# Nicolo2277/Vivim

Hardware: AMD Instinct MI355X
Metric: frames/sec fwd+bwd, 256x256 clip=5 3-class (higher is better)
Workload: dtype bf16

## Files before the change

### vivim_amd/csrc/scan_bwd.hip

```cpp
#include "scan_plan.cuh"

namespace vivim {

constexpr int kBwdWaves = 4;

template <typename T, int K, int R, bool HAS_Z, bool VAR_BC, bool DET = false>
__global__ void __launch_bounds__(kBwdWaves * kWave) ssm_bwd_generic_kernel(const vivim_ssm_bwd_params p, const int ck) {
    constexpr int TILE = kWave * K;
    const vivim_ssm_fwd_params& f = p.f;
    const int lane = threadIdx.x & 63;
    const int wave = threadIdx.x >> 6;
    const int b = blockIdx.y;
    const int N = f.dstate, L = f.seqlen;
    const int cpg = f.dim / f.n_groups;
    const int wpg = (cpg + R - 1) / R;
    const int ws = blockIdx.x * kBwdWaves + wave;
    if (ws >= wpg * f.n_groups) return;
    const int g = ws / wpg;
    const int d0 = g * cpg + (ws - g * wpg) * R;
    const int nvalid = min(R, (g + 1) * cpg - d0);

    extern __shared__ __attribute__((aligned(16))) float smem[];
    constexpr bool FOLD_BC = DET && !VAR_BC;
    float* gcarry = smem + wave * (FOLD_BC ? 5 : 3) * R * N;
// ... 394 lines not shown
                    H = f2{H0, H1};
                }
                {
                    const f2 hend = fma2(P, hck, H);
                    f2 h = dpp_mov2<kDppWaveShr1>(hck, hend);
#pragma unroll
                    for (int k = 0; k < K; ++k) {
                        h = fma2(a[k], h, wB[k]);
                        hs[k] = h;
                    }
                }
                const f2 an = dpp_mov2<kDppWaveShl1>(afirst, a[0]);
                f2 cdy[K], Pr = an, G = {0.0f, 0.0f};
#pragma unroll
                for (int k = K - 1; k >= 0; --k) {
                    const f2 al = k == K - 1 ? an : a[k + 1];
                    cdy[k] = dy[k] * Cn[k];
                    G = fma2(al, G, cdy[k]);
                    if (k < K - 1) Pr *= al;
                }
                f2 gfirst;
                {
                    float P0 = Pr.x, G0 = G.x, P1 = Pr.y, G1 = G.y;
                    wave_scan2_affine_rev_rows(P0, G0, P1, G1);
                    wave_scan_rev_join(P0, G0, lane);
                    wave_scan_rev_join(P1, G1, lane);
                    gfirst = fma2(f2{P0, P1}, gcar, f2{G0, G1});
                }
                f2 gc = dpp_mov2<kDppWaveShl1>(gcar, gfirst);
                f2 dA_part = {0.0f, 0.0f};
                float dBv[K], dCv[K];
#pragma unroll
                for (int k = K - 1; k >= 0; --k) {
                    const f2 al = k == K - 1 ? an : a[k + 1];
                    gc = fma2(al, gc, cdy[k]);
                    const f2 t = gc * (hs[k] - wB[k]);
                    S1[k] = fma2(gc, f2{Bn[k], Bn[k]}, S1[k]);
                    S2[k] = fma2(t, a2v, S2[k]);
                    dA_part = fma2(t, dl[k], dA_part);
                    const f2 db = gc * w[k], dc = dy[k] * hs[k];
                    dBv[k] = db.x + db.y;
                    dCv[k] = dc.x + dc.y;
                }
                if (DA_LDS) {
                    dAl[n * kWave + lane] += dA_part;
                    if (lane == 0) {
                        f2* qq = reinterpret_cast<f2*>(rec + n * kRec * R);
                        qq[GCAR] = gfirst;
                        qq[AFIRST] = a[0];
                    }
                } else {
                    const float dA0 = read_lane(wave_sum_dpp_to63(dA_part.x), 63);
                    const float dA1 = read_lane(wave_sum_dpp_to63(dA_part.y), 63);
                    if (lane == 0) {
                        f2* qq = reinterpret_cast<f2*>(rec + n * kRec * R);
                        qq[GCAR] = gfirst;
                        qq[AFIRST] = a[0];
                        qq[DAACC] += f2{dA0, dA1};
                    }
                }
                {
                    float* sl = slots + ((n & (NBUF - 1)) * W + wave) * SLOT + lane;
#pragma unroll
                    for (int k = 0; k < K; ++k) {
                        sl[k * kWave] = dBv[k];
                        sl[(K + k) * kWave] = dCv[k];
                    }
                }
                lds_barrier();
#pragma unroll
                for (int j = 0; j < EPT; ++j) {
                    const int e = tid + j * (W * kWave);
                    const int e_tok = e & (TILE - 1), e_isC = e / TILE;
                    const float* sp = slots + (n & (NBUF - 1)) * W * SLOT +
                                      (e_isC * K + (e_tok & (K - 1))) * kWave + (e_tok / K);
                    float acc = sp[0];
#pragma unroll
                    for (int wv = 1; wv < W; ++wv) acc += sp[wv * SLOT];
                    const int tq = step * TILE + e_tok;
                    const int t = tq < L ? tq : tq % L;
                    if (DET) {
                        if (tq < L) (e_isC ? dCg + n * p.dC_dstate_stride : dBg + n * p.dB_dstate_stride)[tq] = acc;
                        continue;
                    }
                    atomicAdd((e_isC ? dCg + n * p.dC_dstate_stride : dBg + n * p.dB_dstate_stride) + t, acc);
                }
            }
        }
#pragma unroll
        for (int r = 0; r < R; ++r) {
            float duv[K], ddv[K], uu[K];
            unpack(load_vec_always<T, K>(uB + d[r] * f.u_d_stride + t0, in, uB + d[r] * f.u_d_stride), uu);
#pragma unroll
            for (int k = 0; k < K; ++k) {
                duv[k] = fmaf(dl[k][r], S1[k][r], Dv[r] * dy[k][r]);
                ddv[k] = fmaf(uu[k], S1[k][r], S2[k][r] * kLn2);
            }
            if (f.delta_softplus) {
                float df[K];
                unpack(load_vec_always<T, K>(dlB + d[r] * f.delta_d_stride + t0, in, dlB + d[r] * f.delta_d_stride), df);
#pragma unroll
                for (int k = 0; k < K; ++k) {
                    const float raw = df[k] + bias[r];
                    if (raw <= 20.0f) ddv[k] *= sigmoidf_fast(raw);
                }
            }
#pragma unroll
            for (int k = 0; k < K; ++k) dbias_acc[r] += in ? ddv[k] : 0.0f;
            store_vec<T, K>(static_cast<T*>(p.du) + b * p.du_batch_stride + d[r] * p.du_d_stride + t0, in && active && r < nvalid, duv);
            store_vec<T, K>(static_cast<T*>(p.ddelta) + b * p.ddelta_batch_stride + d[r] * p.ddelta_d_stride + t0, in && active && r < nvalid, ddv);
        }
    }
    if (active) {
#pragma unroll
        for (int r = 0; r < R; ++r) {
            if (r >= nvalid) break;
            const float sD = wave_sum(dD_acc[r]);
            const float sb = wave_sum(dbias_acc[r]);
            if (lane == 0) {
                const int64_t slot = DET ? (int64_t)(b * gridDim.z + seg) * f.dim : 0;
                if (p.dD) det_add<DET>(static_cast<float*>(p.dD) + slot + d[r], sD);
                if (p.ddelta_bias) det_add<DET>(static_cast<float*>(p.ddelta_bias) + slot + d[r], sb);
            }
        }
        wave_lds_fence();
        for (int i = lane; i < N * R; i += kWave) {
            const int n = i / R, r = i - n * R;
            float tot = VIVIM_REC(n, DAACC, r);
            if (DA_LDS) {
                const float* q = reinterpret_cast<const float*>(dAl + n * kWave) + r;
                tot = 0.0f;
                for (int j = 0; j < kWave; ++j) tot += q[j * R];
            }
            if (r < nvalid)
                det_add<DET>(static_cast<float*>(p.dA) + (DET ? (int64_t)(b * gridDim.z + seg) * f.dim * N : 0) +
                             (d0 + r) * p.dA_d_stride + n * p.dA_dstate_stride, tot);
        }
    }
#undef VIVIM_REC
}

constexpr int kPreW = 4;
template <typename T, int K, bool HAS_Z, int NS>
__global__ void __launch_bounds__(kPreW * kWave) ssm_bwd_prepass_kernel(const vivim_ssm_bwd_params p, const BwdSeg sg) {
    constexpr int R = kBwR;
    constexpr int TILE = kWave * K;
    const vivim_ssm_fwd_params& f = p.f;
    const int lane = threadIdx.x & 63;
    const int wave = __builtin_amdgcn_readfirstlane(threadIdx.x >> 6);
    const int b = blockIdx.y;
    const int N = f.dstate, L = f.seqlen;
    const int cpg = f.dim / f.n_groups;
    const int ppg = (cpg + R - 1) / R;
    const int nw = blockDim.x >> 6;
    const int bpg = (ppg + nw - 1) / nw;
    const int g = blockIdx.x / bpg;
    const int pair = (blockIdx.x - g * bpg) * nw + wave;
    if (pair >= ppg) return;
    const int d0 = g * cpg + pair * R;
    const int nvalid = min(R, (g + 1) * cpg - d0);
    const int nsteps = (L + TILE - 1) / TILE;
    const int seg = blockIdx.z + 1;
    const int s_lo = seg * sg.seg_steps, s_hi = min(nsteps, s_lo + sg.seg_steps);
    const int t_next = s_hi * TILE;

    extern __shared__ __attribute__((aligned(16))) float smem[];
    float* acc = smem + wave * (N * R * kWave);
    if (NS == 0)
        for (int i = lane; i < N * R * kWave; i += kWave) acc[i] = 0.0f;
    f2 racc[NS > 0 ? NS : 1];
#pragma unroll
    for (int n = 0; n < (NS > 0 ? NS : 1); ++n) racc[n] = f2{0.0f, 0.0f};

    int d[R];
    float bias[R], a2v[R];
#pragma unroll
    for (int r = 0; r < R; ++r) {
        d[r] = d0 + min(r, nvalid - 1);
        bias[r] = f.delta_bias ? static_cast<const float*>(f.delta_bias)[d[r]] : 0.0f;
        a2v[r] = lane < N ? static_cast<const float*>(f.A)[d[r] * f.A_d_stride + lane * f.A_dstate_stride] * kLog2e : 0.0f;
    }
    const T* __restrict__ dlB = static_cast<const T*>(f.delta) + b * f.delta_batch_stride;
    const T* __restrict__ doB = static_cast<const T*>(p.dout) + b * p.dout_batch_stride;
    const T* __restrict__ zB = HAS_Z ? static_cast<const T*>(f.z) + b * f.z_batch_stride : nullptr;
    const T* __restrict__ Cv = static_cast<const T*>(f.C) + b * f.C_batch_stride + g * f.C_group_stride;
    wave_lds_fence();

    float base[R] = {0.0f, 0.0f}, dfirst[R] = {0.0f, 0.0f};
    RawK<T, K> ndl[R], ndo[R], nz[R];
    auto request = [&](int step) __attribute__((always_inline)) {
        const int t0 = step * TILE + lane * K;
        const bool in = step < s_hi && t0 < L;
#pragma unroll
        for (int r = 0; r < R; ++r) {
            ndl[r] = load_vec_always<T, K>(dlB + d[r] * f.delta_d_stride + t0, in, dlB + d[r] * f.delta_d_stride);
            ndo[r] = load_vec_always<T, K>(doB + d[r] * p.dout_d_stride + t0, in, doB + d[r] * p.dout_d_stride);
            if (HAS_Z) nz[r] = load_vec_always<T, K>(zB + d[r] * f.z_d_stride + t0, in, zB + d[r] * f.z_d_stride);
        }
    };
    constexpr bool kAhead = sizeof(T) * K <= 16;
    if (kAhead) request(s_lo);
    for (int step = s_lo; step < s_hi; ++step) {
        const int t0 = step * TILE + lane * K;
        const bool in = t0 < L;
        float c[R][K], dy[R][K];
        RawK<T, K> cdl[R], cdo[R], cz[R];
        if (!kAhead) request(step);
#pragma unroll
        for (int r = 0; r < R; ++r) { cdl[r] = ndl[r]; cdo[r] = ndo[r]; if (HAS_Z) cz[r] = nz[r]; }
        if (kAhead) request(step + 1);
#pragma unroll
        for (int r = 0; r < R; ++r) {
            float df[K];
            unpack(cdl[r], df);
            unpack(cdo[r], dy[r]);
            if (HAS_Z) {
                float zf[K];
                unpack(cz[r], zf);
#pragma unroll
                for (int k = 0; k < K; ++k) dy[r][k] *= zf[k] * sigmoidf_fast(zf[k]);
            }
            float run = 0.0f;
#pragma unroll
            for (int k = 0; k < K; ++k) {
                const float raw = df[k] + bias[r];
                const float sp = f.delta_softplus ? softplus_ref(raw) : raw;
                run += in ? sp : 0.0f;
                c[r][k] = run;
            }
            if (step == s_lo) {
                dfirst[r] = read_lane(c[r][0], 0);
                base[r] = -dfirst[r];
            }
            const float incl = wave_sum_dpp_to63(run);
            const float off = incl - run + base[r];
#pragma unroll
            for (int k = 0; k < K; ++k) c[r][k] += off;
            base[r] += read_lane(incl, 63);
        }
        RawK<T, K> Craw = load_vec_always<T, K>(Cv + t0, in, Cv);
        if (NS > 0) {
            f2 cp[K], dyp[K];
#pragma unroll
            for (int k = 0; k < K; ++k) { cp[k] = f2{c[0][k], c[1][k]}; dyp[k] = f2{dy[0][k], dy[1][k]}; }
#pragma unroll
            for (int n = 0; n < NS; ++n) {
                float Cn[K];
                unpack(Craw, Cn);
                Craw = load_vec_always<T, K>(Cv + (n + 1) * f.C_dstate_stride + t0, in && (n + 1 < NS), Cv);
                const f2 A2 = {read_lane(a2v[0], n), read_lane(a2v[1], n)};
#pragma unroll
                for (int k = 0; k < K; ++k) racc[n] = fma2(exp2_2(A2 * cp[k]), dyp[k] * Cn[k], racc[n]);
            }
        } else {
#pragma unroll 1
            for (int n = 0; n < N; ++n) {
                float Cn[K];
                unpack(Craw, Cn);
                Craw = load_vec_always<T, K>(Cv + (n + 1) * f.C_dstate_stride + t0, in && (n + 1 < N), Cv);
#pragma unroll
                for (int r = 0; r < R; ++r) {
                    const float A2 = read_lane(a2v[r], n);
                    float* q = acc + (n * R + r) * kWave + lane;
                    float v = *q;
#pragma unroll
                    for (int k = 0; k < K; ++k) v = fmaf(fast_exp2(A2 * c[r][k]), Cn[k] * dy[r][k], v);
                    *q = v;
                }
            }
        }
    }
    if (NS > 0) {
#pragma unroll
        for (int n = 0; n < NS; ++n) {
            acc[(n * R + 0) * kWave + lane] = racc[n].x;
            acc[(n * R + 1) * kWave + lane] = racc[n].y;
        }
    }
    wave_lds_fence();
    for (int row0 = 0; row0 < N * R; row0 += kWave / 2) {
        const int row = row0 + (lane >> 1);
        float v = 0.0f;
        if (row < N * R) {
            const float* q = acc + row * kWave + (lane & 1) * (kWave / 2);
#pragma unroll 8
            for (int j = 0; j < kWave / 2; ++j) v += q[j];
        }
        v += __shfl_xor(v, 1, kWave);
        const int n = row / R, r = row - n * R;
        if (row < N * R && (lane & 1) == 0 && r < nvalid)
            sg.agg[(((int64_t)b * f.dim + d0 + r) * sg.S + seg) * N + n] = v;
    }
#pragma unroll
    for (int r = 0; r < R; ++r) {
        float dl_nx = 0.0f;
        if (t_next < L) {
            const float raw = to_f32<T>((dlB + d[r] * f.delta_d_stride)[t_next]) + bias[r];
            dl_nx = f.delta_softplus ? softplus_ref(raw) : raw;
        }
        if (lane == 0 && r < nvalid) sg.dsum[((int64_t)b * f.dim + d[r]) * sg.S + seg] = base[r] + dl_nx;
    }
}

__global__ void ssm_bwd_carry_kernel(const vivim_ssm_bwd_params p, const BwdSeg sg) {
    const vivim_ssm_fwd_params& f = p.f;
    const int64_t i = (int64_t)blockIdx.x * blockDim.x + threadIdx.x;
    const int N = f.dstate;
    if (i >= (int64_t)f.batch * f.dim * N) return;
    const int n = (int)(i % N);
    const int64_t bd = i / N;
    const int dch = (int)(bd % f.dim);
    const float A2 = static_cast<const float*>(f.A)[dch * f.A_d_stride + n * f.A_dstate_stride] * kLog2e;
    float g = 0.0f;
    const int S = sg.S;
    sg.gin[(bd * S + S - 1) * N + n] = 0.0f;
    for (int i0 = 0; i0 < S - 1; i0 += 8) {
        float ag[8], ds[8];
#pragma unroll
        for (int q = 0; q < 8; ++q) {
            const int s = S - 1 - (i0 + q);
            const bool ok = s >= 1;
            ag[q] = ok ? sg.agg[(bd * S + s) * N + n] : 0.0f;
            ds[q] = ok ? sg.dsum[bd * S + s] : 0.0f;
        }
#pragma unroll
        for (int q = 0; q < 8; ++q) {
            const int s = S - 1 - (i0 + q);
            if (s >= 1) {
                g = fmaf(fast_exp2(A2 * ds[q]), g, ag[q]);
                sg.gin[(bd * S + s - 1) * N + n] = g;
            }
        }
    }
}

template <typename T, int K, int DS>
static void launch_prepass(const vivim_ssm_bwd_params& p, const BwdSeg& sg, hipStream_t stream) {
    const vivim_ssm_fwd_params& f = p.f;
    const int ppg = (f.dim / f.n_groups + kBwR - 1) / kBwR;
    const size_t per_wave = (size_t)f.dstate * kBwR * kWave * sizeof(float);
    int nw = (int)((size_t)65536 / per_wave);
    nw = nw > kPreW ? kPreW : (nw < 1 ? 1 : nw);
    const dim3 gpre(((ppg + nw - 1) / nw) * f.n_groups, f.batch, sg.S - 1);
    if (f.z) hipLaunchKernelGGL((ssm_bwd_prepass_kernel<T, K, true, DS>), gpre, dim3(nw * kWave), nw * per_wave, stream, p, sg);
    else     hipLaunchKernelGGL((ssm_bwd_prepass_kernel<T, K, false, DS>), gpre, dim3(nw * kWave), nw * per_wave, stream, p, sg);
    const int64_t nthr = (int64_t)f.batch * f.dim * f.dstate;
    hipLaunchKernelGGL(ssm_bwd_carry_kernel, dim3((unsigned)((nthr + 255) / 256)), dim3(256), 0, stream, p, sg);
}

void launch_bwd_closed_prepass(const vivim_ssm_bwd_params& p, const LsSeg& ls, int K, hipStream_t stream) {
    const BwdSeg sg = {ls.S, ls.seg_blocks * 16 / (K * kWave), ls.agg, ls.dsum, ls.gin};
    with_itype(p.f.itype, [&](auto t) {
        typedef decltype(t) T;
        if (K == 8) launch_prepass<T, 8, 16>(p, sg, stream); else launch_prepass<T, 4, 16>(p, sg, stream);
    });
}

template <typename T, int K, int W, bool DET>
static void launch_bwd_fast_kw(const vivim_ssm_bwd_params& p, const BwdPlan& q, hipStream_t stream) {
    const vivim_ssm_fwd_params& f = p.f;
    const int ppg = (f.dim / f.n_groups + kBwR - 1) / kBwR;
    const int bpg = (ppg + W - 1) / W;
    BwdSeg sg = {q.S, q.seg, nullptr, nullptr, nullptr};
    if (q.S > 1) {
        const size_t nbd = (size_t)f.batch * f.dim * sg.S;
        sg.agg = static_cast<float*>(p.workspace);
        sg.gin = sg.agg + nbd * f.dstate;
        sg.dsum = sg.gin + nbd * f.dstate;
        if (f.dstate == 16) launch_prepass<T, K, 16>(p, sg, stream);
        else                launch_prepass<T, K, 0>(p, sg, stream);
    }
    const size_t smem = ((size_t)2 * W * 2 * K * kWave + (size_t)W * f.dstate * kBwR * kRec +
                         (q.da_lds ? (size_t)W * f.dstate * kWave * 2 : 0)) * sizeof(float);
    const dim3 grid(bpg * f.n_groups, f.batch, sg.S), block(W * kWave);
    auto launch = [&](auto kernel) {
        allow_smem(kernel, smem);
        hipLaunchKernelGGL(kernel, grid, block, smem, stream, p, sg);
    };
    if (f.z) { if (q.da_lds) launch(ssm_bwd_fast_kernel<T, K, true, W, true, DET>); else launch(ssm_bwd_fast_kernel<T, K, true, W, false, DET>); }
    else     { if (q.da_lds) launch(ssm_bwd_fast_kernel<T, K, false, W, true, DET>); else launch(ssm_bwd_fast_kernel<T, K, false, W, false, DET>); }
}

template <bool DET>
static void launch_bwd_fast_t(const vivim_ssm_bwd_params& p, const BwdPlan& q, hipStream_t stream) {
    with_itype(p.f.itype, [&](auto t) {
        typedef decltype(t) T;
        if (q.K == 8) {
            if constexpr (DET) launch_bwd_fast_kw<T, 8, 4, DET>(p, q, stream);
            else if (q.W == 4) launch_bwd_fast_kw<T, 8, 4, DET>(p, q, stream);
            else               launch_bwd_fast_kw<T, 8, kBwWmax, DET>(p, q, stream);
        }
        else          { if (q.W == 4) launch_bwd_fast_kw<T, 4, 4, DET>(p, q, stream); else launch_bwd_fast_kw<T, 4, kBwWmax, DET>(p, q, stream); }
    });
}
void launch_bwd_fast(const vivim_ssm_bwd_params& p, const BwdPlan& q, hipStream_t stream, bool det) {
    if (det) launch_bwd_fast_t<true>(p, q, stream); else launch_bwd_fast_t<false>(p, q, stream);
}

template <bool DET>
static void launch_bwd_generic_t(const vivim_ssm_bwd_params& p, int ck, hipStream_t stream) {
    constexpr int K = 4, R = kBwdGenR;
    const vivim_ssm_fwd_params& f = p.f;
    const int sets = ((f.dim / f.n_groups + R - 1) / R) * f.n_groups;
    const dim3 grid((sets + kBwdWaves - 1) / kBwdWaves, f.batch), block(kBwdWaves * kWave);
    const bool var = f.is_variable_B;
    const size_t smem = (size_t)kBwdWaves * (DET && !var ? 5 : 3) * R * f.dstate * sizeof(float);
    with_itype(f.itype, [&](auto t) {
        typedef decltype(t) T;
        if (f.z) {
            if (var) hipLaunchKernelGGL((ssm_bwd_generic_kernel<T, K, R, true, true, DET>), grid, block, smem, stream, p, ck);
            else     hipLaunchKernelGGL((ssm_bwd_generic_kernel<T, K, R, true, false, DET>), grid, block, smem, stream, p, ck);
        } else {
            if (var) hipLaunchKernelGGL((ssm_bwd_generic_kernel<T, K, R, false, true, DET>), grid, block, smem, stream, p, ck);
            else     hipLaunchKernelGGL((ssm_bwd_generic_kernel<T, K, R, false, false, DET>), grid, block, smem, stream, p, ck);
        }
    });
}
void launch_bwd_generic(const vivim_ssm_bwd_params& p, int ck, hipStream_t stream, bool det) {
    if (det) launch_bwd_generic_t<true>(p, ck, stream); else launch_bwd_generic_t<false>(p, ck, stream);
}

}
```

### vivim_amd/csrc/scan_plan.hip

```cpp
#include <stdlib.h>
#include <algorithm>
#include <atomic>
#include "scan_plan.cuh"

namespace vivim {

const ScanEnv& scan_env() {
    static const ScanEnv e = [] {
        auto num = [](const char* name, int dflt) { const char* v = getenv(name); return v ? atoi(v) : dflt; };
        return ScanEnv{num("VIVIM_CHAN_WAVES", 2048), num("VIVIM_CHAN_XCD", -1)};
    }();
    return e;
}

static int cu_count() {
    static const int n = [] {
        int dev = 0, v = 0;
        if (hipGetDevice(&dev) != hipSuccess ||
            hipDeviceGetAttribute(&v, hipDeviceAttributeMultiprocessorCount, dev) != hipSuccess || v <= 0)
            v = 256;
        return v;
    }();
    return n;
}

static int ls_bwd_blocks_per_cu(const vivim_ssm_fwd_params& f, int W, bool ls2) {
    static std::atomic<int> cache[2][3][3][2][5];
    if (f.itype < 0 || f.itype > 2) return ls2 ? 2 : 3;
    std::atomic<int>& c = cache[ls2][f.itype][f.dstate / 32][f.z != nullptr][W];
    int nb = c.load(std::memory_order_relaxed);
    if (nb == 0) {
        nb = ls2 ? ls2_bwd_occupancy(f, W) : ls_bwd_occupancy(f, W);
        c.store(nb, std::memory_order_relaxed);
    }
    return nb;
}

static bool rows_vec_ok(const void* ptr, std::initializer_list<int64_t> strides, int64_t epv, int es) {
    if (reinterpret_cast<uintptr_t>(ptr) % (uintptr_t)(epv * es)) return false;
    for (int64_t s : strides)
        if (s % epv) return false;
    return true;
}
static int esize(int itype) { return itype == VIVIM_F32 ? 4 : 2; }
static int epv16(int itype) { return 16 / esize(itype); }
static bool fwd_rows_vec_ok(const vivim_ssm_fwd_params& f, int64_t epv, bool ptrs = true) {
    const int es = esize(f.itype);
    auto P = [&](const void* q) { return ptrs ? q : nullptr; };
    return rows_vec_ok(P(f.u), {f.u_batch_stride, f.u_d_stride}, epv, es) &&
           rows_vec_ok(P(f.delta), {f.delta_batch_stride, f.delta_d_stride}, epv, es) &&
           rows_vec_ok(P(f.out), {f.out_batch_stride, f.out_d_stride}, epv, es) &&
           (!f.z || (rows_vec_ok(P(f.z), {f.z_batch_stride, f.z_d_stride}, epv, es) &&
                     rows_vec_ok(P(f.out_z), {f.out_z_batch_stride, f.out_z_d_stride}, epv, es)));
}
static bool b_rows_vec_ok(const vivim_ssm_fwd_params& f, int64_t epv) {
    return rows_vec_ok(f.B, {f.B_batch_stride, f.B_group_stride, f.B_dstate_stride}, epv, esize(f.itype));
}
static bool c_rows_vec_ok(const vivim_ssm_fwd_params& f, int64_t epv) {
    return rows_vec_ok(f.C, {f.C_batch_stride, f.C_group_stride, f.C_dstate_stride}, epv, esize(f.itype));
}
static bool bwd_rows_vec_ok(const vivim_ssm_bwd_params& p, int64_t epv) {
    const vivim_ssm_fwd_params& f = p.f;
    const int es = esize(f.itype);
    return rows_vec_ok(f.u, {f.u_batch_stride, f.u_d_stride}, epv, es) &&
           rows_vec_ok(f.delta, {f.delta_batch_stride, f.delta_d_stride}, epv, es) &&
           rows_vec_ok(p.dout, {p.dout_batch_stride, p.dout_d_stride}, epv, es) &&
           rows_vec_ok(p.du, {p.du_batch_stride, p.du_d_stride}, epv, es) &&
           rows_vec_ok(p.ddelta, {p.ddelta_batch_stride, p.ddelta_d_stride}, epv, es) &&
           (!f.z || (rows_vec_ok(f.z, {f.z_batch_stride, f.z_d_stride}, epv, es) &&
                     rows_vec_ok(f.out, {f.out_batch_stride, f.out_d_stride}, epv, es) &&
                     rows_vec_ok(p.dz, {p.dz_batch_stride, p.dz_d_stride}, epv, es) &&
                     (!f.out_z || rows_vec_ok(f.out_z, {f.out_z_batch_stride, f.out_z_d_stride}, epv, es))));
}

static bool ls_span_ok(int64_t rows, int64_t row_stride, int64_t len, int es) {
    return row_stride >= 0 && ((rows - 1) * row_stride + len) * es < (int64_t)0xffff0000;
}
static bool ls_shape_ok(const vivim_ssm_fwd_params& f) {
    if (!(f.is_variable_B && f.is_variable_C && (f.dstate == 16 || f.dstate == 32 || f.dstate == 64) && f.dim % f.n_groups == 0))
        return false;
    const int es = esize(f.itype);
    if (f.dim > 65520 || !ls_span_ok(f.dim, f.u_d_stride, f.seqlen, es) || !ls_span_ok(f.dim, f.delta_d_stride, f.seqlen, es) ||
        !ls_span_ok(f.dstate, f.B_dstate_stride, f.seqlen, es) || !ls_span_ok(f.dstate, f.C_dstate_stride, f.seqlen, es) ||
        !ls_span_ok(f.dim, (int64_t)((f.seqlen + 15) / 16) * f.dstate, 0, 4))
        return false;
    if (f.z && (!ls_span_ok(f.dim, f.z_d_stride, f.seqlen, es))) return false;
    return true;
}
static int ls_ckpt_len(const vivim_ssm_fwd_params& f) { return 16 * (f.dstate / 16); }

static bool ls_rows(const vivim_ssm_fwd_params& f) {
    if (!ls_shape_ok(f)) return false;
    const int t = tuning_fwd_variant();
    if (t == kFwdChan || t == kFwdStates) return true;
    if (t != kFwdAuto) return false;
    return f.dstate == 16 && f.seqlen <= (f.itype == VIVIM_F32 ? 8192 : 32768);
}

int scan_ckpt_len(const vivim_ssm_fwd_params& f) { return ls_rows(f) ? ls_ckpt_len(f) : kChunk; }
int scan_chunk_len(int) { return kChunk; }

static void ls_segmentation(const vivim_ssm_fwd_params& f, int waves_per_seg, int slots, int min_blocks, int& S, int& seg_blocks) {
    const int nck = (f.seqlen + ls_ckpt_len(f) - 1) / ls_ckpt_len(f);
    int s = slots / waves_per_seg;
    const int smax = nck / min_blocks;
    if (s > smax) s = smax;
    if (s > 512) s = 512;
    if (s < 1) s = 1;
    seg_blocks = (nck + s - 1) / s;
    S = (nck + seg_blocks - 1) / seg_blocks;
}
static size_t seg_ws_bytes(const vivim_ssm_fwd_params& f, int S) {
    return S > 1 ? (size_t)f.batch * f.dim * S * (2 * f.dstate + 1) * sizeof(float) : 0;
}
static bool ws_ok(const void* ws, int64_t bytes, size_t need) { return need && ws && (size_t)bytes >= need; }

static bool chan_shape_ok(const vivim_ssm_fwd_params& f, int ck) {
    if (!f.is_variable_B || !f.is_variable_C || (f.dstate != 16 && f.dstate != 64) || f.seqlen % 8 != 0) return false;
    if (f.dim % f.n_groups != 0 || (f.dim / f.n_groups) % kWave != 0) return false;
    const int tune = tuning_fwd_variant();
    if (tune != kFwdChan) {
        if (tune != kFwdAuto) return false;
        if (f.dstate == 64 && f.itype == VIVIM_F32) return false;
        const int64_t cols = (int64_t)f.batch * (f.dim / kWave);
        const int64_t least = ck < kChunk ? 150000 : 110000;
        if (cols < 8 || cols * f.seqlen < least) return false;
    }
    return fwd_rows_vec_ok(f, epv16(f.itype), false);
}
static size_t chan_layout(const vivim_ssm_fwd_params& f, FwdPlan& q) {
    const int tt = f.itype == VIVIM_F32 ? ChTile<float>::TT : ChTile<bf16_t>::TT;
    const int ntiles = (f.seqlen + tt - 1) / tt;
    const int64_t waves = (int64_t)((f.dim / f.n_groups + kWave - 1) / kWave) * f.n_groups * f.batch;
    int64_t want = (scan_env().chan_waves + waves - 1) / waves;
    if (want > ntiles) want = ntiles;
    if (want > 512) want = 512;
    if (want < 1) want = 1;
    q.seg = (int)((ntiles + want - 1) / want);
    q.S = (ntiles + q.seg - 1) / q.seg;
    q.Lpad = ntiles * tt;
    q.bc_floats = (size_t)f.batch * f.n_groups * (q.Lpad + 1) * 32 * (f.dstate / 16);
    const size_t h_floats = q.S > 1 ? (size_t)f.batch * f.dim * q.S * (f.dstate + 1) : 0;
    return (q.bc_floats + h_floats) * sizeof(float);
}
static void ls_fwd_segmentation(const vivim_ssm_fwd_params& f, int& S, int& seg_blocks) {
    const int cpw = (4 / (f.dstate / 16)) * kLsCPR;
    const int cpg = f.dim / f.n_groups;
    const int waves_per_seg = ((cpg + 4 * cpw - 1) / (4 * cpw)) * 4 * f.n_groups * f.batch;
    ls_segmentation(f, waves_per_seg, cu_count() * 28, 4, S, seg_blocks);
}

static FwdPlan plan_scan_fwd(const vivim_ssm_fwd_params& f, bool launch) {
    FwdPlan q{};
    const bool states = ls_rows(f);
    q.ck = states ? ls_ckpt_len(f) : kChunk;
    const bool chan = chan_shape_ok(f, q.ck);
    const size_t chan_ws = chan ? chan_layout(f, q) : 0;
    int lsS = 1, ls_seg = 0;
    if (states) ls_fwd_segmentation(f, lsS, ls_seg);
    const size_t ls_ws = states ? seg_ws_bytes(f, lsS) : 0;
    q.ws = chan_ws > ls_ws ? chan_ws : ls_ws;
    if (!launch) return q;

    if (chan && fwd_rows_vec_ok(f, epv16(f.itype)) && f.workspace && (size_t)f.workspace_bytes >= chan_ws &&
        (reinterpret_cast<uintptr_t>(f.workspace) & 63) == 0) {
        const int wg_per_group = ((f.dim / f.n_groups) / kWave + kChWaves - 1) / kChWaves;
        q.xcd = scan_env().chan_xcd >= 0 ? scan_env().chan_xcd : ((wg_per_group >= 2 || f.itype != VIVIM_F32) ? 1 : 0);
        q.family = FwdFamily::chan;
        return q;
    }
    if (states) {
        const int es = esize(f.itype);
        if (!ls_span_ok(f.dim, f.out_d_stride, f.seqlen, es) || (f.z && !ls_span_ok(f.dim, f.out_z_d_stride, f.seqlen, es)))
            return q;
        q.family = FwdFamily::states;
        q.bc_vec = b_rows_vec_ok(f, epv16(f.itype)) && c_rows_vec_ok(f, epv16(f.itype));
        const bool seg = ws_ok(f.workspace, f.workspace_bytes, ls_ws);
        q.S = seg ? lsS : 1;
        q.seg = seg ? ls_seg : (f.seqlen + q.ck - 1) / q.ck;
        return q;
    }
    q.family = FwdFamily::generic;
    const int epv = epv16(f.itype);
    if (!f.is_variable_B || !f.is_variable_C || f.dstate % 8 != 0 || f.seqlen % 8 != 0 || !fwd_rows_vec_ok(f, epv) ||
        !b_rows_vec_ok(f, epv) || !c_rows_vec_ok(f, epv))
        return q;
    const int t = tuning_fwd_variant();
    const int64_t nwg = (int64_t)((f.dim / f.n_groups + kNsR - 1) / kNsR) * f.n_groups * f.batch;
    const int v = (t != kFwdAuto && t < kFwdChan) ? t : ((nwg >= 512 && f.seqlen < 4096) ? kFwdNsplitK4 : kFwdNsplitK8);
    if (v == kFwdGeneric) return q;
    q.family = FwdFamily::nsplit;
    q.K = v == kFwdNsplitK4 ? 4 : 8;
    return q;
}

size_t scan_fwd_workspace_bytes(const vivim_ssm_fwd_params& f) { return plan_scan_fwd(f, false).ws; }

bool ssm_fwd_dispatch(const vivim_ssm_fwd_params& p, hipStream_t s) {
    const FwdPlan q = plan_scan_fwd(p, true);
    switch (q.family) {
        case FwdFamily::chan: launch_fwd_chan(p, q, s); return true;
        case FwdFamily::states: launch_ls_fwd(p, q, s); return true;
        case FwdFamily::nsplit: launch_fwd_nsplit(p, q, s); return true;
        case FwdFamily::generic: launch_fwd_generic(p, s); return true;
        case FwdFamily::none: break;
    }
    return false;
}

static int ls_bwd_waves(const vivim_ssm_fwd_params& f) {
    const int cpw = (4 / (f.dstate / 16)) * kLsCPR;
    const int w = (f.dim / f.n_groups + cpw - 1) / cpw;
    return w > 4 ? 4 : w;
}

static int bwd_tokens_per_lane(int seqlen) {
    const int64_t slots8 = (int64_t)((seqlen + 511) / 512) * 512, slots4 = (int64_t)((seqlen + 255) / 256) * 256;
    return slots8 * 100 > slots4 * 115 ? 4 : 8;
}

static int64_t bwd_segmentation(const vivim_ssm_fwd_params& f, int K, int W, int& S, int& seg_steps) {
    const int tile = kWave * K;
    const int nsteps = (f.seqlen + tile - 1) / tile;
    const int ppg = (f.dim / f.n_groups + kBwR - 1) / kBwR;
    const int64_t base = (int64_t)((ppg + W - 1) / W) * f.n_groups * f.batch;
    const int slots = cu_count() * (K == 4 && W == 4 ? 3 : kBwWmax / W);
    int best = 1;
    double best_cost = 1e300;
    for (int s = 1; s <= nsteps && s <= 64; ++s) {
        const int steps = (nsteps + s - 1) / s;
        if ((nsteps + steps - 1) / steps != s) continue;
        const double rounds = (double)((base * s + slots - 1) / slots);
        const double cost = rounds * (steps * (1.0 + 0.4 * (s - 1) / s) + 0.3);
        if (cost < best_cost - 1e-9) { best_cost = cost; best = s; }
    }
    seg_steps = (nsteps + best - 1) / best;
    S = (nsteps + seg_steps - 1) / seg_steps;
    return base * S;
}

static BwdPlan plan_scan_bwd(const vivim_ssm_fwd_params& f, const vivim_ssm_bwd_params* p) {
    BwdPlan q{};
    q.ck = scan_ckpt_len(f);
    const int tv = tuning_bwd_variant();
    if (ls_shape_ok(f) && q.ck == ls_ckpt_len(f) && (tv == kBwdAuto || tv == kBwdStates1 || tv == kBwdStates2)) {
        const bool ls2_wanted = f.dstate == 16 && f.seqlen % epv16(f.itype) == 0 && (tv == kBwdAuto || tv == kBwdStates2);
        q.W = ls_bwd_waves(f);
        const int cpw = (4 / (f.dstate / 16)) * kLsCPR;
        const int bpg = (f.dim / f.n_groups + q.W * cpw - 1) / (q.W * cpw);
        ls_segmentation(f, bpg * q.W * f.n_groups * f.batch, cu_count() * ls_bwd_blocks_per_cu(f, q.W, ls2_wanted) * q.W, 4,
                        q.S, q.seg);
        const int nck = (f.seqlen + 15) / 16;
        if (ls2_wanted && q.S > 1 && q.seg >= 12) {
            q.seg = (q.seg + 8) / 16 * 16;
            q.S = (nck + q.seg - 1) / q.seg;
        }
        q.ws = seg_ws_bytes(f, q.S);
        if (!p) return q;
        q.family = BwdFamily::generic;
        {
            const int es = esize(f.itype);
            if (f.x == nullptr || !ls_span_ok(f.dim, p->dout_d_stride, f.seqlen, es) ||
                !ls_span_ok(f.dim, p->du_d_stride, f.seqlen, es) || !ls_span_ok(f.dim, p->ddelta_d_stride, f.seqlen, es))
                return q;
            if (f.z && (!ls_span_ok(f.dim, f.out_d_stride, f.seqlen, es) || !ls_span_ok(f.dim, p->dz_d_stride, f.seqlen, es) ||
                        (f.out_z && !ls_span_ok(f.dim, f.out_z_d_stride, f.seqlen, es))))
                return q;
        }
        q.family = BwdFamily::states;
        if (!ws_ok(p->workspace, p->workspace_bytes, q.ws)) {
            q.S = 1;
            q.seg = (f.seqlen + ls_ckpt_len(f) - 1) / ls_ckpt_len(f);
        }
        const int epv = epv16(f.itype);
        q.bc_vec = b_rows_vec_ok(f, epv) && c_rows_vec_ok(f, epv);
        q.ls2 = ls2_wanted && bwd_rows_vec_ok(*p, epv);
        q.K = (q.seg * 16) % 512 == 0 && f.seqlen % 8 == 0 ? 8 : 4;
        const int es = esize(f.itype), pv = (q.K * es >= 16 ? 16 : q.K * es) / es;
        q.closed_prepass = q.S > 1 && q.ls2 && (q.seg * 16) % 256 == 0 && f.seqlen % q.K == 0 &&
                           rows_vec_ok(f.delta, {f.delta_batch_stride, f.delta_d_stride}, pv, es) &&
                           rows_vec_ok(p->dout, {p->dout_batch_stride, p->dout_d_stride}, pv, es) &&
                           (!f.z || rows_vec_ok(f.z, {f.z_batch_stride, f.z_d_stride}, pv, es)) && c_rows_vec_ok(f, pv);
        return q;
    }
    if (f.is_variable_B && f.is_variable_C && f.dstate <= 64) {
        q.K = bwd_tokens_per_lane(f.seqlen);
        q.W = kBwWmax;
        const int64_t wgs = bwd_segmentation(f, q.K, q.W, q.S, q.seg);
        if (tv == kBwdTokensW4 || (tv != kBwdTokensW8 && (wgs > cu_count() || q.seg >= 4))) {
            q.W = 4;
            bwd_segmentation(f, q.K, q.W, q.S, q.seg);
        }
        q.ws = seg_ws_bytes(f, q.S);
    }
    if (!p) return q;
    q.family = BwdFamily::generic;
    const int es = esize(f.itype), epv = (q.K * es >= 16 ? 16 : q.K * es) / es;
    if (!q.K || f.x == nullptr || tv == kBwdGeneric || q.ck != kChunk || f.seqlen % q.K != 0 || !bwd_rows_vec_ok(*p, epv) ||
        !b_rows_vec_ok(f, epv) || !c_rows_vec_ok(f, epv))
        return q;
    q.family = BwdFamily::tokens;
    if (!ws_ok(p->workspace, p->workspace_bytes, q.ws)) {
        q.S = 1;
        q.seg = (f.seqlen + kWave * q.K - 1) / (kWave * q.K);
    }
    q.da_lds = f.dstate <= 16 && q.seg >= 2;
    return q;
}

size_t scan_bwd_workspace_bytes(const vivim_ssm_fwd_params& f) { return plan_scan_bwd(f, nullptr).ws; }

static void det_tokens_width(const vivim_ssm_fwd_params& f, const vivim_ssm_bwd_params* p, BwdPlan& q) {
    if (q.K != 8 || q.W != kBwWmax) return;
    q.W = 4;
    bwd_segmentation(f, q.K, q.W, q.S, q.seg);
    q.ws = seg_ws_bytes(f, q.S);
    if (p && q.family == BwdFamily::tokens) {
        if (!ws_ok(p->workspace, p->workspace_bytes, q.ws)) {
            q.S = 1;
            q.seg = (f.seqlen + kWave * q.K - 1) / (kWave * q.K);
        }
        q.da_lds = f.dstate <= 16 && q.seg >= 2;
    }
}

struct ScanDetLayout {
    int64_t nA, nB, eB;
    size_t bytes;
};
static ScanDetLayout scan_det_layout(const vivim_ssm_fwd_params& f, BwdFamily fam, int S, int W) {
    const int64_t cpg = f.dim / f.n_groups, bgnl = (int64_t)f.batch * f.n_groups * f.dstate * f.seqlen;
    ScanDetLayout l{(int64_t)f.batch, 0, 0, 0};
    if (fam == BwdFamily::generic) {
        l.nB = f.is_variable_B ? (cpg + kBwdGenR - 1) / kBwdGenR : f.batch;
        l.eB = f.is_variable_B ? bgnl : (int64_t)f.dim * f.dstate;
    } else if (fam == BwdFamily::tokens) {
        l.nA = (int64_t)f.batch * S;
        l.nB = ((cpg + kBwR - 1) / kBwR + W - 1) / W;
        l.eB = bgnl;
    } else {
        const int64_t cpb = (int64_t)W * (4 / (f.dstate / 16)) * kLsCPR, bpg = (cpg + cpb - 1) / cpb;
        l.nA = (int64_t)f.batch * S;
        l.nB = bpg > 2 ? bpg : 0;
        l.eB = bpg > 2 ? bgnl : 0;
    }
    l.bytes = sizeof(float) * (size_t)(l.nA * f.dim * (f.dstate + 2) + 2 * l.nB * l.eB);
    return l;
}

size_t scan_bwd_det_workspace_bytes(const vivim_ssm_fwd_params& f) {
    BwdPlan q = plan_scan_bwd(f, nullptr);
    det_tokens_width(f, nullptr, q);
    const size_t gen = scan_det_layout(f, BwdFamily::generic, 1, 0).bytes;
    if (!q.W) return gen;
    const BwdFamily fam = q.K ? BwdFamily::tokens : BwdFamily::states;
    return std::max(gen, scan_det_layout(f, fam, q.S, q.W).bytes);
}

size_t scan_bwd_det_call_workspace_bytes(const vivim_ssm_bwd_params& p) {
    BwdPlan q = plan_scan_bwd(p.f, &p);
    if (q.family == BwdFamily::none) return 0;
    det_tokens_width(p.f, &p, q);
    return scan_det_layout(p.f, q.family, q.S, q.W).bytes;
}

int ssm_bwd_det_dispatch(const vivim_ssm_bwd_params& p, void* det_ws, size_t det_ws_bytes, hipStream_t s) {
    const vivim_ssm_fwd_params& f = p.f;
    BwdPlan q = plan_scan_bwd(f, &p);
    if (q.family == BwdFamily::none) return 1;
    det_tokens_width(f, &p, q);
    const ScanDetLayout l = scan_det_layout(f, q.family, q.S, q.W);
    if (det_ws == nullptr || det_ws_bytes < l.bytes || reinterpret_cast<uintptr_t>(det_ws) % 16 != 0) return 2;
    float* wA = static_cast<float*>(det_ws);
    float* wD = wA + l.nA * f.dim * f.dstate;
    float* wb = wD + l.nA * f.dim;
    float* wB = wb + l.nA * f.dim;
    float* wC = wB + l.nB * l.eB;
    vivim_ssm_bwd_params d = p;
    d.dA = wA; d.dA_d_stride = f.dstate; d.dA_dstate_stride = 1;
    if (p.dD) d.dD = wD;
    if (p.ddelta_bias) d.ddelta_bias = wb;
    const bool varBC = f.is_variable_B;
    if (l.nB) {
        d.dB = wB; d.dC = wC;
        if (varBC) {
            d.dB_batch_stride = d.dC_batch_stride = (int64_t)f.n_groups * f.dstate * f.seqlen;
            d.dB_group_stride = d.dC_group_stride = (int64_t)f.dstate * f.seqlen;
            d.dB_dstate_stride = d.dC_dstate_stride = f.seqlen;
        } else {
            d.dB_batch_stride = d.dC_batch_stride = 0;
            d.dB_group_stride = d.dC_group_stride = f.dstate;
            d.dB_dstate_stride = d.dC_dstate_stride = 1;
        }
    }
    switch (q.family) {
        case BwdFamily::states: launch_ls_bwd(d, q, s, true); break;
        case BwdFamily::tokens: launch_bwd_fast(d, q, s, true); break;
        case BwdFamily::generic: launch_bwd_generic(d, q.ck, s, true); break;
        case BwdFamily::none: return 1;
    }
    det_reduce(wA, (int)l.nA, det_out(static_cast<float*>(p.dA), {f.dim, f.dstate}, {p.dA_d_stride, p.dA_dstate_stride}), s);
    if (p.dD) det_reduce(wD, (int)l.nA, det_out(static_cast<float*>(p.dD), {f.dim}, {1}), s);
    if (p.ddelta_bias) det_reduce(wb, (int)l.nA, det_out(static_cast<float*>(p.ddelta_bias), {f.dim}, {1}), s);
    if (l.nB) {
        auto bc = [&](float* w, void* out, int64_t bs, int64_t gs, int64_t ns) {
            if (varBC) det_reduce(w, (int)l.nB, det_out(static_cast<float*>(out), {f.batch, f.n_groups, f.dstate, f.seqlen}, {bs, gs, ns, 1}), s);
            else       det_reduce(w, (int)l.nB, det_out(static_cast<float*>(out), {f.dim, f.dstate}, {gs, ns}), s);
        };
        bc(wB, p.dB, p.dB_batch_stride, p.dB_group_stride, p.dB_dstate_stride);
        bc(wC, p.dC, p.dC_batch_stride, p.dC_group_stride, p.dC_dstate_stride);
    }
    return 0;
}

bool ssm_bwd_dispatch(const vivim_ssm_bwd_params& p, hipStream_t s) {
    const BwdPlan q = plan_scan_bwd(p.f, &p);
    switch (q.family) {
        case BwdFamily::states: launch_ls_bwd(p, q, s); return true;
        case BwdFamily::tokens: launch_bwd_fast(p, q, s); return true;
        case BwdFamily::generic: launch_bwd_generic(p, q.ck, s); return true;
        case BwdFamily::none: break;
    }
    return false;
}

}
```

Before: 185.6.

## Add dedicated bf16 segment-aggregate kernel for closed backward prepass

Adds a new ssm_seg_agg_kernel that computes per-segment state aggregates and delta sums for 16-bit inputs. It processes channel pairs packed into float2, prefetches the next tile's delta, dout, z and C, and reduces across the wave through LDS plus DPP. Several segments can be assigned to one wavefront (ipw) to balance the grid. For 2-byte types the closed prepass now uses this kernel with K=4 instead of the generic prepass, and the planner forces K=4 for non-fp32. The aim is fewer redundant loads and better occupancy in the backward prepass, at the cost of a new specialised code path restricted to dstate 16.

```diff
diff --git a/vivim_amd/csrc/scan_bwd.hip b/vivim_amd/csrc/scan_bwd.hip
--- a/vivim_amd/csrc/scan_bwd.hip
+++ b/vivim_amd/csrc/scan_bwd.hip
@@ -720,6 +720,164 @@
     }
 }
 
+constexpr int kAggW = 4;
+constexpr int kAggRS = 72;
+typedef float f4 __attribute__((ext_vector_type(4)));
+template <typename T, bool HAS_Z>
+__global__ void __launch_bounds__(kAggW * kWave) ssm_seg_agg_kernel(const vivim_ssm_bwd_params p, const BwdSeg sg, const int ipw) {
+    constexpr int R = kBwR, K = 4, NS = 16;
+    constexpr int TILE = kWave * K;
+    static_assert(R == 2 && sizeof(T) == 2, "packed channel pairs, 8-byte vectors of 4 tokens");
+    const vivim_ssm_fwd_params& f = p.f;
+    const int lane = threadIdx.x & 63;
+    const int wave = __builtin_amdgcn_readfirstlane(threadIdx.x >> 6);
+    const int b = blockIdx.y;
+    const int L = f.seqlen;
+    const int cpg = f.dim / f.n_groups;
+    const int ppg = (cpg + R - 1) / R;
+    const int bpg = (ppg + kAggW - 1) / kAggW;
+    const int g = blockIdx.x / bpg;
+    const int pair = (blockIdx.x - g * bpg) * kAggW + wave;
+    if (pair >= ppg) return;
+    const int d0 = g * cpg + pair * R;
+    const int nvalid = min(R, (g + 1) * cpg - d0);
+    const int nsteps = (L + TILE - 1) / TILE;
+    const int seg_lo = 1 + blockIdx.z * ipw;
+    const int s_lo = seg_lo * sg.seg_steps, s_hi = min(nsteps, min(sg.S, seg_lo + ipw) * sg.seg_steps);
+    if (s_lo >= s_hi) return;
+
+    __shared__ __attribute__((aligned(16))) f2 red_all[kAggW * NS * kAggRS];
+    f2* red = red_all + wave * (NS * kAggRS);
+
+    int d[R];
+    float bias[R], a2v[R];
+#pragma unroll
+    for (int r = 0; r < R; ++r) {
+        d[r] = d0 + min(r, nvalid - 1);
+        bias[r] = f.delta_bias ? static_cast<const float*>(f.delta_bias)[d[r]] : 0.0f;
+        a2v[r] = lane < NS ? static_cast<const float*>(f.A)[d[r] * f.A_d_stride + lane * f.A_dstate_stride] * kLog2e : 0.0f;
+    }
+    f2 A2[NS];
+#pragma unroll
+    for (int n = 0; n < NS; ++n) A2[n] = f2{read_lane(a2v[0], n), read_lane(a2v[1], n)};
+    const T* __restrict__ dlB = static_cast<const T*>(f.delta) + b * f.delta_batch_stride;
+    const T* __restrict__ doB = static_cast<const T*>(p.dout) + b * p.dout_batch_stride;
+    const T* __restrict__ zB = HAS_Z ? static_cast<const T*>(f.z) + b * f.z_batch_stride : nullptr;
+    const T* __restrict__ Cv = static_cast<const T*>(f.C) + b * f.C_batch_stride + g * f.C_group_stride;
+
+    RawK<T, K> ndl[R], ndo[R], nz[R];
+    auto request = [&](int step) __attribute__((always_inline)) {
+        const int t0 = step * TILE + lane * K;
+        const bool in = step < s_hi && t0 < L;
+        const bool ind = t0 < L && (step < s_hi || lane == 0);
+#pragma unroll
+        for (int r = 0; r < R; ++r) {
+            ndl[r] = load_vec_always<T, K>(dlB + d[r] * f.delta_d_stride + t0, ind, dlB + d[r] * f.delta_d_stride);
+            ndo[r] = load_vec_always<T, K>(doB + d[r] * p.dout_d_stride + t0, in, doB + d[r] * p.dout_d_stride);
+            if (HAS_Z) nz[r] = load_vec_always<T, K>(zB + d[r] * f.z_d_stride + t0, in, zB + d[r] * f.z_d_stride);
+        }
+    };
+    request(s_lo);
+    auto load_c = [&](int n, int t) __attribute__((always_inline)) {
+        union { u32x2 v; RawK<T, K> r; } u;
+        u.v = *reinterpret_cast<const u32x2*>(Cv + n * f.C_dstate_stride + t);
+        return u.r;
+    };
+    RawK<T, K> Cr[NS];
+#pragma unroll
+    for (int n = 0; n < NS; ++n) Cr[n] = load_c(n, min(s_lo * TILE + lane * K, L - K));
+    f2 racc[NS];
+#pragma unroll
+    for (int n = 0; n < NS; ++n) racc[n] = f2{0.0f, 0.0f};
+    float base[R] = {0.0f, 0.0f};
+    int sis = 0;
+    for (int step = s_lo; step < s_hi; ++step) {
+        const int t0 = step * TILE + lane * K;
+        const bool in = t0 < L;
+        const int tc_nx = step + 1 < s_hi ? min(t0 + TILE, L - K) : 0;
+        RawK<T, K> cdl[R], cdo[R], cz[R];
+#pragma unroll
+        for (int r = 0; r < R; ++r) { cdl[r] = ndl[r]; cdo[r] = ndo[r]; if (HAS_Z) cz[r] = nz[r]; }
+        request(step + 1);
+        float c[R][K], dy[R][K];
+#pragma unroll
+        for (int r = 0; r < R; ++r) {
+            float df[K];
+            unpack(cdl[r], df);
+            unpack(cdo[r], dy[r]);
+            if (HAS_Z) {
+                float zf[K];
+                unpack(cz[r], zf);
+#pragma unroll
+                for (int k = 0; k < K; ++k) dy[r][k] *= zf[k] * sigmoidf_fast(zf[k]);
+            }
+            float run = 0.0f;
+#pragma unroll
+            for (int k = 0; k < K; ++k) {
+                const float raw = df[k] + bias[r];
+                const float sp = f.delta_softplus ? softplus_ref(raw) : raw;
+                run += in ? sp : 0.0f;
+                c[r][k] = run;
+            }
+            if (sis == 0) base[r] = -read_lane(c[r][0], 0);
+            const float incl = wave_sum_dpp_to63(run);
+            const float off = incl - run + base[r];
+#pragma unroll
+            for (int k = 0; k < K; ++k) c[r][k] += off;
+            base[r] += read_lane(incl, 63);
+        }
+        f2 cp[K], dyp[K];
+#pragma unroll
+        for (int k = 0; k < K; ++k) { cp[k] = f2{c[0][k], c[1][k]}; dyp[k] = f2{dy[0][k], dy[1][k]}; }
+#pragma unroll
+        for (int n = 0; n < NS; ++n) {
+            float Cn[K];
+            {
+                union { RawK<T, K> r; u32x2 v; } cr;
+                cr.r = Cr[n];
+                asm volatile("" : "+v"(cr.v));
+                unpack(cr.r, Cn);
+            }
+            Cr[n] = load_c(n, tc_nx);
+            __builtin_amdgcn_sched_barrier(0);
+#pragma unroll
+            for (int k = 0; k < K; ++k) racc[n] = fma2(exp2_2(A2[n] * cp[k]), dyp[k] * Cn[k], racc[n]);
+        }
+        ++sis;
+        if (sis == sg.seg_steps || step + 1 == nsteps) {
+            const int seg = step / sg.seg_steps;
+#pragma unroll
+            for (int n = 0; n < NS; ++n) { red[n * kAggRS + lane] = racc[n]; racc[n] = f2{0.0f, 0.0f}; }
+            wave_lds_fence();
+            {
+                const int n = lane >> 2, q = lane & 3;
+                const f2* src = red + n * kAggRS + 2 * q;
+                f2 s = {0.0f, 0.0f};
+#pragma unroll
+                for (int i = 0; i < kWave / 8; ++i) {
+                    const f4 v = *reinterpret_cast<const f4*>(src + 8 * i);
+                    s += f2{v.x, v.y};
+                    s += f2{v.z, v.w};
+                }
+                s.x += dpp_mov<0xB1>(0.0f, s.x);
+                s.y += dpp_mov<0xB1>(0.0f, s.y);
+                s.x += dpp_mov<0x4E>(0.0f, s.x);
+                s.y += dpp_mov<0x4E>(0.0f, s.y);
+                if (q < nvalid) sg.agg[(((int64_t)b * f.dim + d0 + q) * sg.S + seg) * NS + n] = q == 0 ? s.x : s.y;
+            }
+            wave_lds_fence();
+            const bool has_nx = (step + 1) * TILE < L;
+#pragma unroll
+            for (int r = 0; r < R; ++r) {
+                const float raw = to_f32<T>(ndl[r].e[0]) + bias[r];
+                const float dl_nx = has_nx ? read_lane(f.delta_softplus ? softplus_ref(raw) : raw, 0) : 0.0f;
+                if (lane == 0 && r < nvalid) sg.dsum[((int64_t)b * f.dim + d[r]) * sg.S + seg] = base[r] + dl_nx;
+            }
+            sis = 0;
+        }
+    }
+}
+
 __global__ void ssm_bwd_carry_kernel(const vivim_ssm_bwd_params p, const BwdSeg sg) {
     const vivim_ssm_fwd_params& f = p.f;
     const int64_t i = (int64_t)blockIdx.x * blockDim.x + threadIdx.x;
@@ -767,10 +925,26 @@
 }
 
 void launch_bwd_closed_prepass(const vivim_ssm_bwd_params& p, const LsSeg& ls, int K, hipStream_t stream) {
-    const BwdSeg sg = {ls.S, ls.seg_blocks * 16 / (K * kWave), ls.agg, ls.dsum, ls.gin};
-    with_itype(p.f.itype, [&](auto t) {
+    const vivim_ssm_fwd_params& f = p.f;
+    with_itype(f.itype, [&](auto t) {
         typedef decltype(t) T;
-        if (K == 8) launch_prepass<T, 8, 16>(p, sg, stream); else launch_prepass<T, 4, 16>(p, sg, stream);
+        if constexpr (sizeof(T) == 2) {
+            const BwdSeg sg = {ls.S, ls.seg_blocks * 16 / (4 * kWave), ls.agg, ls.dsum, ls.gin};
+            const int ppg = (f.dim / f.n_groups + kBwR - 1) / kBwR;
+            const int bpg = (ppg + kAggW - 1) / kAggW;
+            const int64_t items = (int64_t)bpg * kAggW * f.n_groups * f.batch * (sg.S - 1);
+            int ipw = (int)std::min<int64_t>(8, std::max<int64_t>(1, items / 8192));
+            const int chunks = (sg.S - 1 + ipw - 1) / ipw;
+            ipw = (sg.S - 1 + chunks - 1) / chunks;
+            const dim3 grid(bpg * f.n_groups, f.batch, chunks);
+            if (f.z) hipLaunchKernelGGL((ssm_seg_agg_kernel<T, true>), grid, dim3(kAggW * kWave), 0, stream, p, sg, ipw);
+            else     hipLaunchKernelGGL((ssm_seg_agg_kernel<T, false>), grid, dim3(kAggW * kWave), 0, stream, p, sg, ipw);
+            const int64_t nthr = (int64_t)f.batch * f.dim * f.dstate;
+            hipLaunchKernelGGL(ssm_bwd_carry_kernel, dim3((unsigned)((nthr + 255) / 256)), dim3(256), 0, stream, p, sg);
+        } else {
+            const BwdSeg sg = {ls.S, ls.seg_blocks * 16 / (K * kWave), ls.agg, ls.dsum, ls.gin};
+            if (K == 8) launch_prepass<T, 8, 16>(p, sg, stream); else launch_prepass<T, 4, 16>(p, sg, stream);
+        }
     });
 }
 
diff --git a/vivim_amd/csrc/scan_plan.hip b/vivim_amd/csrc/scan_plan.hip
--- a/vivim_amd/csrc/scan_plan.hip
+++ b/vivim_amd/csrc/scan_plan.hip
@@ -275,8 +275,9 @@
         const int epv = epv16(f.itype);
         q.bc_vec = b_rows_vec_ok(f, epv) && c_rows_vec_ok(f, epv);
         q.ls2 = ls2_wanted && bwd_rows_vec_ok(*p, epv);
-        q.K = (q.seg * 16) % 512 == 0 && f.seqlen % 8 == 0 ? 8 : 4;
-        const int es = esize(f.itype), pv = (q.K * es >= 16 ? 16 : q.K * es) / es;
+        const int es = esize(f.itype);
+        q.K = es == 4 && (q.seg * 16) % 512 == 0 && f.seqlen % 8 == 0 ? 8 : 4;
+        const int pv = (q.K * es >= 16 ? 16 : q.K * es) / es;
         q.closed_prepass = q.S > 1 && q.ls2 && (q.seg * 16) % 256 == 0 && f.seqlen % q.K == 0 &&
                            rows_vec_ok(f.delta, {f.delta_batch_stride, f.delta_d_stride}, pv, es) &&
                            rows_vec_ok(p->dout, {p->dout_batch_stride, p->dout_d_stride}, pv, es) &&
```

New measurement: 178.1. -4.0%, worse.
